# MatthewRalston/kmerdb

Measured on AMD Instinct MI355X. Metric: k-mers counted/sec at k=12, synthetic 150 bp FASTQ, higher is better.
Workload: dtype u64

## Files before the change

### kmerdb_amd/csrc/kdb_engine.hip

```cpp
#include <hip/hip_runtime.h>

#include <cmath>
#include <cstdarg>
#include <cstddef>
#include <cstdio>
#include <cstdlib>
#include <algorithm>
#include <atomic>
#include <cstring>
#include <string>
#include <thread>
#include <vector>

#include "../../include/kdbhip.h"
#include "kdb_kernels.hip.h"
#include "kdb_hist.hip.h"
#include "kdb_scatter.hip.h"
#include "kdb_scatter_host.hip.h"
#include "kdb_smallk.hip.h"
#include "kdb_probe.hip.h"
#include "kdb_gram.hip.h"
#include "kdb_pairstats.hip.h"
#include "kdb_sizefactors.hip.h"
#include "kdb_spectrum.hip.h"
// ... 67 lines not shown
struct kdb_engine {
    int k = 0, canonical = 1, n_mode = KDB_N_DROP, device = 0;
    uint64_t nbins = 0;
    unsigned long long *d_table = nullptr;
    bool owns_table = false;
    bool table_escaped = false;
    kdb::DevCounters *d_ctr = nullptr;
    unsigned long long *d_worklist = nullptr;
    size_t worklist_cap = 1u << 20;
    uint32_t *d_first_rec = nullptr; size_t first_rec_cap = 0;
    unsigned long long *d_suspects = nullptr;
    unsigned long long *sh_suspects = nullptr;
    size_t suspects_cap = 1u << 16;
    hipStream_t s_compute = nullptr, s_copy = nullptr;

    size_t stage_bytes = 64ull << 20, stage_reads = 2ull << 20;
    uint8_t *h_bases[NBUF] = {nullptr, nullptr};
    uint64_t *h_offs[NBUF] = {nullptr, nullptr};
    uint8_t *d_bases[NBUF] = {nullptr, nullptr};
    uint64_t *d_offs[NBUF] = {nullptr, nullptr};
    hipEvent_t ev_copied[NBUF] = {nullptr, nullptr}, ev_done[NBUF] = {nullptr, nullptr};
    bool inflight[NBUF] = {false, false};
    hipEvent_t busy[NBUF] = {nullptr, nullptr};
    int next_buf = 0;
    bool staging_ready = false;
    int copy_threads = 8;

    int64_t accum_bytes = -1;
    size_t acc_cap = 0, acc_reads_cap = 0;
    uint8_t *d_acc_bases[2] = {nullptr, nullptr};
    uint64_t *d_acc_offs[2] = {nullptr, nullptr};
    hipEvent_t ev_acc_done[2] = {nullptr, nullptr};
    hipEvent_t ev_acc_copied = nullptr;
    hipEvent_t ev_pin[2] = {nullptr, nullptr};
    bool pin_used[2] = {false, false};
    int pin_idx = 0;
    bool acc_inflight[2] = {false, false};
    int acc_slot = 0;
    size_t acc_nb = 0, acc_nr = 0;
    bool acc_ready = false;

    int64_t algo = 0;
    int min_len = 0;
    int smallk_old = 0;
    kdb::PagedOptions opt;
    kdb::ScatterState sc;
    int overlap = 0;
    int overlap_hist_cus = 0;
    int overlap_mask_mode = 0;
    bool compute_masked = false;
    hipStream_t s_hist = nullptr;
    kdb::OverlapState ov;
    kdb::TwoLevelPaged tp;
    int64_t oom_fallbacks = 0;
    int strand_merge = 1;
    int strand_merge_max_k = 12;
    unsigned long long *d_fwd = nullptr;
    bool strands_pending = false;

    bool tableless = false;
    uint8_t *sh_seq = nullptr; size_t sh_seq_cap = 0;
    uint64_t *sh_offs = nullptr; size_t sh_offs_cap = 0;
    unsigned long long *sh_ids = nullptr; size_t sh_ids_cap = 0;
    kdb::DevCounters *sh_ctr = nullptr;

    unsigned long long *d_acc_table = nullptr;
    uint64_t folded_files = 0, folded_total = 0;
    uint64_t d2h_bytes = 0;
    uint64_t bytes_in = 0;

    bool prof = false;
    std::vector<ProfSpan> spans;
    std::vector<hipEvent_t> ev_pool;
    double prof_ms[KDB_N_KERNELS] = {0};
    uint64_t prof_n[KDB_N_KERNELS] = {0};
};

namespace {

struct DeviceGuard {
    int prev = -1;
    explicit DeviceGuard(int dev) { if (hipGetDevice(&prev) != hipSuccess) prev = -1; (void)hipSetDevice(dev); }
    ~DeviceGuard() { if (prev >= 0) (void)hipSetDevice(prev); }
};

hipEvent_t prof_event(kdb_engine *e)
{
    hipEvent_t ev = nullptr;
    if (!e->ev_pool.empty()) { ev = e->ev_pool.back(); e->ev_pool.pop_back(); return ev; }
    if (hipEventCreate(&ev) != hipSuccess) return nullptr;
    return ev;
}

struct ProfScope {
    kdb_engine *e; int kernel; hipStream_t stream; hipEvent_t a = nullptr, b = nullptr;
    ProfScope(kdb_engine *e_, int kernel_, hipStream_t stream_ = nullptr) : e(e_), kernel(kernel_), stream(stream_ ? stream_ : e_->s_compute)
    {
        if (!e->prof) return;
        a = prof_event(e); b = prof_event(e);
        if (a) (void)hipEventRecord(a, stream);
    }
    ~ProfScope()
    {
        if (!e->prof || !a || !b) return;
        (void)hipEventRecord(b, stream);
        e->spans.push_back({a, b, kernel});
// ... 167 lines not shown
        ProfScope ps(e, KDB_KERNEL_MARK);
        const unsigned ug = (unsigned)std::min<uint64_t>((nreads + 255) / 256, 4096);
        hipLaunchKernelGGL(kdb::unmark_reads_kernel, dim3(ug), dim3(256), 0, e->s_compute, d_bases, d_offs, (uint64_t)nreads, first_is_continuation,
                           (const kdb::DevCounters *)e->d_ctr);
        marked = false;
    };
    bool no_first_rec = false;
    {
        const size_t need = ((nbytes >> kdb::FIRST_REC_SHIFT) + 2) * sizeof(uint32_t);
        if (e->first_rec_cap < need && e->d_first_rec) HIP_TRY(hipStreamSynchronize(e->s_compute));
        int grc = grow((void **)&e->d_first_rec, &e->first_rec_cap, need);
        if (grc == KDB_ERR_NOMEM) no_first_rec = true;
        else if (grc != KDB_OK) return grc;
    }
    {
        ProfScope ps(e, KDB_KERNEL_MARK);
        const dim3 grid((unsigned)((nreads + 255) / 256)), block(256);
        HIP_TRY(hipMemsetAsync(&e->d_ctr->neg_min_len, 0, kdb::PER_BATCH_WORDS * sizeof(unsigned long long), e->s_compute));
        const dim3 lgrid(grid.x < 1024u ? grid.x : 1024u);
        hipLaunchKernelGGL(kdb::lens_kernel, lgrid, block, 0, e->s_compute, d_offs, (uint64_t)nreads, (uint64_t)nbytes,
                           e->min_len > 0 ? e->min_len : e->k, first_is_continuation, e->d_ctr, e->d_first_rec);
    }
    if (nbytes == 0) return KDB_OK;
    if (nreads > 0xFFFFFFF0ull) return fail(KDB_ERR_ARG, "batch of %zu records: at most 2^32 - 16 per submit", nreads);
    e->bytes_in += nbytes;
    const kdb::RecStarts rs{d_offs, e->d_first_rec, (uint32_t)nreads, first_is_continuation ? 1u : 0u};
    int algo = (int)e->algo;
    if (algo == 0 || algo == 3) algo = 2;
    if (no_first_rec && algo == 2) { algo = 1; e->oom_fallbacks++; e->tp.table_is_zero = false; }
    const bool paged2 = algo == 2 && e->k > e->opt.one_level_max_k;
    if (!paged2 || e->n_mode == KDB_N_EXPAND || !e->opt.defer) e->tp.table_is_zero = false;
    const bool staged = e->canonical && e->strand_merge && algo == 2 && e->k <= std::min((int)e->opt.one_level_max_k, e->strand_merge_max_k) &&
                        !e->overlap && !e->smallk_old && ensure_fwd(e);
    const int canonical = staged ? 0 : e->canonical;
    unsigned long long *const table = staged ? e->d_fwd : e->d_table;
    if (staged) e->strands_pending = true;
    if (algo == 2) {
        EngineProf hook(e);
        const bool ex = e->n_mode == KDB_N_EXPAND;
        const kdb::ScBatch batch{d_bases, nbytes, rs, e->k, canonical, ex, table, e->d_ctr};
        int rc;
        if (e->k <= kdb::SMALLK_LDS_MAX_K && !e->smallk_old)
            rc = kdb::smallk_lds_count(e->s_compute, d_bases, nbytes, rs, e->k, canonical, ex, e->opt.grid, table, e->d_ctr, hook);
        else if (e->k <= kdb::SMALLK_MAX) {
            mark();
            rc = kdb::smallk_count(e->s_compute, d_bases, nbytes, e->k, canonical, ex, table, e->d_ctr, hook);
            unmark();
        }
        else if (e->k <= e->opt.one_level_max_k) {
            rc = 3;
            if (e->overlap && e->s_hist && !ex) rc = kdb::scatter_count_overlapped(e->ov, e->opt, e->s_compute, e->s_hist, batch, hook);
            if (rc == 3) {
                { const int jrc = overlap_join(e); if (jrc != KDB_OK) return jrc; }
                rc = kdb::scatter_count(e->sc, e->opt, e->s_compute, batch, hook);
            }
        }
        else {
            const size_t lost = nreads * (size_t)(e->k - 1);
            rc = kdb::twolevel_paged_count(e->tp, e->opt, e->s_compute, batch, nbytes > lost ? nbytes - lost : 0, hook);
        }
        if (rc == 2) { e->oom_fallbacks++; algo = 1; e->tp.table_is_zero = false; }
        else if (rc != 0) return fail(KDB_ERR_HIP, "LDS-histogram path failed: %s", kdb::partition_error());
    }
    if (algo == 1) {
        { const int jrc = overlap_join(e); if (jrc != KDB_OK) return jrc; }
        mark();
        {
            ProfScope ps(e, KDB_KERNEL_COUNT);
            const bool ex = (e->n_mode == KDB_N_EXPAND);
            const dim3 grid((unsigned)ntiles), block(kdb::TPB);
#define KDB_LAUNCH_DIRECT(ID, EX)                                                                              \
    hipLaunchKernelGGL((kdb::count_direct_kernel<ID, EX>), grid, block, 0, e->s_compute, d_bases, (uint64_t)nbytes, \
                       e->k, canonical, table, e->d_ctr)
            if (e->k <= 16) { if (ex) KDB_LAUNCH_DIRECT(uint32_t, true); else KDB_LAUNCH_DIRECT(uint32_t, false); }
            else            { if (ex) KDB_LAUNCH_DIRECT(uint64_t, true); else KDB_LAUNCH_DIRECT(uint64_t, false); }
#undef KDB_LAUNCH_DIRECT
        }
        unmark();
    }
    if (e->n_mode == KDB_N_EXPAND && e->d_worklist) {
        ProfScope ps(e, KDB_KERNEL_COUNT);
        hipLaunchKernelGGL(kdb::expand_worklist_kernel, dim3(1024), dim3(256), 0, e->s_compute, table, e->d_ctr, e->k, canonical);
    }
    if (e->n_mode == KDB_N_DROP) {
        ProfScope ps(e, KDB_KERNEL_MARK);
        hipLaunchKernelGGL(kdb::resolve_suspects_kernel, dim3(4), dim3(256), 0, e->s_compute, (const uint8_t *)d_bases, (uint64_t)nbytes, d_offs, (uint64_t)nreads,
                           e->k, e->d_ctr);
    }
    HIP_TRY(hipGetLastError());
    return KDB_OK;
}

int flush_pending_paged(kdb_engine *e)
{
    if (e->tp.pending == 0) return KDB_OK;
    EngineProf hook(e);
    if (kdb::twolevel_paged_flush(e->tp, e->opt, e->s_compute, e->d_table, e->d_ctr, hook)) return fail(KDB_ERR_HIP, "LDS-histogram path failed: %s", kdb::partition_error());
    return KDB_OK;
}

int check_errors(kdb_engine *e)
{
    kdb::DevCounters c;
    HIP_TRY(hipMemcpy(&c, e->d_ctr, sizeof c, hipMemcpyDeviceToHost));
    if (c.n_short)
        return fail(KDB_ERR_SHORT_READ, "%llu record(s) shorter than k=%d (reference: kmer.py:461-463 raises)",
                    c.n_short, e->k);
    if (c.bad_layout)
        return fail(KDB_ERR_ARG, "read_offsets must rise from 0 to nbytes (records tile the residue buffer exactly)");
    if (c.internal_err) {
        for (int q = 0; q < 2; q++) {
            unsigned long long hd[2] = {0, 0};
            if (e->ov.side[q] && hipMemcpy(hd, e->ov.side[q], sizeof hd, hipMemcpyDeviceToHost) == hipSuccess && hd[0] > hd[1])
                return fail(KDB_ERR_STATE, "internal: the overlapped path's side list of degenerate ids overflowed (%llu pairs for %llu places); counts are incomplete",
                            hd[0], hd[1]);
        }
        return fail(KDB_ERR_STATE, "internal: a scatter kernel ran out of its page sequence (%llu times); counts are incomplete", c.internal_err);
    }
    if (c.not_uniform)
        return fail(KDB_ERR_ARG, "kdb_submit_device_const needs records of one length (the buffer is never marked); use kdb_submit_device");
    if (c.n_bad)
        return fail(KDB_ERR_BAD_RESIDUE, "%llu residue(s) outside ACGTN%s (reference: kmer.py:309 / :170 raises)", c.n_bad,
                    e->n_mode == KDB_N_DROP ? " that no N in their window shields" : "");
    if (c.marks_seen != c.marks_set)
        return fail(KDB_ERR_BAD_RESIDUE, "the residue buffer holds %lld byte(s) with bit 7 set that are not record starts of their batch "
                                         "(not residues -- kmer.py:170 raises -- or marks left in a device buffer by a job that was aborted)",
                    (long long)(c.marks_seen - c.marks_set));
    return KDB_OK;
}

int grow(void **p, size_t *cap, size_t need_bytes)
{
    if (*cap >= need_bytes) return KDB_OK;
    if (*p) { (void)hipFree(*p); *p = nullptr; *cap = 0; }
    size_t want = need_bytes + need_bytes / 4 + 256;
    hipError_t err = hipMalloc(p, want);
    if (err != hipSuccess) { (void)hipGetLastError(); return fail(KDB_ERR_NOMEM, "hipMalloc(%zu) failed: %s", want, hipGetErrorString(err)); }
    *cap = want;
    return KDB_OK;
}

int shred_scratch(kdb_engine *e, size_t nbytes, size_t nreads)
{
    int rc;
    if ((rc = grow((void **)&e->sh_seq, &e->sh_seq_cap, nbytes + 64)) != KDB_OK) return rc;
    if ((rc = grow((void **)&e->sh_ids, &e->sh_ids_cap, nbytes * 8ull)) != KDB_OK) return rc;
    if (nreads && (rc = grow((void **)&e->sh_offs, &e->sh_offs_cap, (nreads + 1) * sizeof(uint64_t))) != KDB_OK) return rc;
// ... 51 lines not shown
    KDB_PROBE("scatter_64", R_STREAM, W_LINES_SC1, 1, 2),
    KDB_PROBE("scatter_128", R_STREAM, W_CHUNK128_SC1, 1, 2),
    KDB_PROBE("level1_64", R_STREAM, W_LINES_SC1, 1, 3),
    KDB_PROBE("level1_128", R_STREAM, W_CHUNK128_SC1, 1, 3),
    KDB_PROBE("level2_64", R_PAGES15, W_LINES_SC1, 2, 2),
    KDB_PROBE("level2_128", R_PAGES15, W_CHUNK128_SC1, 2, 2),
};
#undef KDB_PROBE
constexpr int N_PROBES = (int)(sizeof(PROBES) / sizeof(PROBES[0]));
}

namespace {
enum OptBefore { OPT_NOTHING, OPT_FLUSH_PENDING , OPT_SYNC_AND_STREAMS ,
                 OPT_SYNC , OPT_NO_STAGING  };
struct OptRow {
    const char *name;
    int64_t (*get)(kdb_engine *);
    void (*set)(kdb_engine *, int64_t) = nullptr;
    bool boolean = false;
    int64_t lo = INT64_MIN, hi = INT64_MAX;
    OptBefore before = OPT_NOTHING;
    const char *hint = "";
    int64_t multiple_of = 1;
};
#define KDB_OPT_RO(field) [](kdb_engine *e) { return (int64_t)e->field; }
#define KDB_OPT(field) KDB_OPT_RO(field), [](kdb_engine *e, int64_t v) { e->field = (decltype(e->field))v; }
const OptRow OPTIONS[] = {
    {"algo", KDB_OPT(algo), false, 0, 3, OPT_NOTHING, " (0 auto, 1 direct atomics, 2 LDS-histogram paths)"},
    {"min_len", KDB_OPT(min_len), false, 0, 64},
    {"copy_threads", KDB_OPT(copy_threads), false, 1, 64},
    {"smallk_old", KDB_OPT(smallk_old), true},
    {"accum_bytes", KDB_OPT(accum_bytes), false, -1, INT64_MAX, OPT_NO_STAGING, " (-1 auto, 0 off, else bytes)"},
    {"stage_bytes", KDB_OPT(stage_bytes), false, 4096, INT64_MAX, OPT_NO_STAGING, " (>=4096, multiple of 16)", 16},
    {"stage_reads", KDB_OPT(stage_reads), false, 1, INT64_MAX, OPT_NO_STAGING},
    {"overlap", KDB_OPT(overlap), true, 0, 1024, OPT_SYNC_AND_STREAMS},
    {"overlap_hist_cus", KDB_OPT(overlap_hist_cus), false, 0, 1024, OPT_SYNC_AND_STREAMS},
    {"overlap_mask_mode", KDB_OPT(overlap_mask_mode), false, 0, 1024, OPT_SYNC_AND_STREAMS},
    {"strand_merge", KDB_OPT(strand_merge), true, 0, 1024, OPT_SYNC},
    {"strand_merge_max_k", KDB_OPT(strand_merge_max_k), false, 1, 17, OPT_SYNC, " (1..17; never more than one_level_max_k)"},
    {"sc_grid", KDB_OPT(opt.grid), false, 0, 1024, OPT_NOTHING, " (0..1024)"},
    {"sc_lo_bits", KDB_OPT(opt.lo_bits), false, 0, kdb::SC_LO_BITS_MAX, OPT_FLUSH_PENDING, " (0 = the default of the path, 1..15)"},
    {"sc_contig_pages", KDB_OPT(opt.contig_pages), true},
    {"sc_wide_lines", KDB_OPT(opt.wide_lines), true},
    {"l1_wide_lines", KDB_OPT(opt.l1_wide), true},
    {"l2_wide_lines", KDB_OPT(opt.l2_wide), true},
    {"l1_one_round", KDB_OPT(opt.l1_one_round), true},
    {"l1_compiled_k", KDB_OPT(opt.l1k), true},
    {"one_level_max_k", KDB_OPT(opt.one_level_max_k), false, 12, kdb::SC1_K, OPT_FLUSH_PENDING, " (12 or 13)"},
    {"defer_flush", KDB_OPT(opt.defer), true},
    {"pending_budget", KDB_OPT(opt.budget_bytes), false, 0, INT64_MAX},
    {"reserve_bytes", KDB_OPT(opt.reserve_bytes), false, 0, INT64_MAX},
    {"arena_grow", KDB_OPT(opt.grow), false, 0, 2, OPT_NOTHING, " (0 never, 1 when it pays, 2 whenever the arena has filled up)"},
    {"arena_batches", KDB_OPT(opt.first_batches), false, 1, kdb::PAGED_PENDING_MAX, OPT_NOTHING, " (1..64: the arena's first size, in batches like the first one)"},
    {"k", KDB_OPT_RO(k)},
    {"arena_budget_bytes", [](kdb_engine *e) { return (int64_t)(e->opt.budget_bytes ? e->opt.budget_bytes : e->tp.budget_decided); }},
    {"free_at_sizing", KDB_OPT_RO(tp.free_at_sizing)},
    {"overlap_scatter_grid", KDB_OPT_RO(ov.grid)},
    {"oom_fallbacks", KDB_OPT_RO(oom_fallbacks)},
    {"pending_batches", KDB_OPT_RO(tp.pending)},
    {"d2h_bytes", KDB_OPT_RO(d2h_bytes)},
    {"folded_files", KDB_OPT_RO(folded_files)},
    {"bytes_in", KDB_OPT_RO(bytes_in)},
    {"arena_pages", KDB_OPT_RO(tp.arena.cap)},
    {"arena_reallocs", KDB_OPT_RO(tp.reallocs)},
    {"hist_flushes", KDB_OPT_RO(tp.flushes)},
    {"flushed_batches", KDB_OPT_RO(tp.flushed_batches)},
    {"full_flushes", KDB_OPT_RO(tp.full_flushes)},
};
#undef KDB_OPT
#undef KDB_OPT_RO
static_assert(kdb::SC_LO_BITS_MAX == 15 && kdb::SC1_K == 13 && kdb::PAGED_PENDING_MAX == 64, "the hints of sc_lo_bits, one_level_max_k and arena_batches spell these out");

const OptRow *find_option(const char *name)
{
    for (const OptRow &row : OPTIONS) if (!strcmp(name, row.name)) return &row;
    return nullptr;
}
}

namespace {

struct GramGroup { uint32_t row0, nrows; int na, nb; bool diag; };

uint32_t gram_grid_max(uint32_t nrows) { return nrows < KDB_GRAM_GRID_MANY_ROWS ? (uint32_t)KDB_GRAM_GRID_MAX : (uint32_t)KDB_GRAM_GRID_MAX_MANY_ROWS; }

void gram_launch(const GramGroup &gr, uint32_t gx, const unsigned long long *const *vecs, const kdbgram::Row *rows, uint32_t nchunks, uint32_t pstride, ulonglong2 *partials,
                 hipStream_t st)
{
    const dim3 grid(gx, gr.nrows), block(kdbgram::TPB);
    const kdbgram::Row *r = rows + gr.row0;
    ulonglong2 *p = partials + (uint64_t)gr.row0 * pstride * kdbgram::NSLOT;
#define KDB_GRAM_CASE(NA, NB, DIAG) hipLaunchKernelGGL((kdbgram::gram_kernel<NA, NB, DIAG>), grid, block, 0, st, vecs, r, nchunks, pstride, p)
    if (gr.diag) {
        switch (gr.na) {
            case 1: KDB_GRAM_CASE(1, 1, true); break;
            case 2: KDB_GRAM_CASE(2, 2, true); break;
            case 3: KDB_GRAM_CASE(3, 3, true); break;
            default: KDB_GRAM_CASE(4, 4, true); break;
        }
    } else {
        switch (gr.nb) {
            case 1: KDB_GRAM_CASE(4, 1, false); break;
            case 2: KDB_GRAM_CASE(4, 2, false); break;
            case 3: KDB_GRAM_CASE(4, 3, false); break;
            default: KDB_GRAM_CASE(4, 4, false); break;
        }
    }
#undef KDB_GRAM_CASE
}

}


extern "C" {

int kdb_abi_version(void) { return KDB_ABI_VERSION; }

const char *kdb_last_error(void) { return g_err.c_str(); }

int kdb_device_count(int *n_out)
// ... 15 lines not shown
    *out = nullptr;
    if (k < 1 || k > 17) return fail(KDB_ERR_ARG, "k=%d outside 1..17 (4^k uint64 table must fit in HBM)", k);
    if (n_mode != KDB_N_DROP && n_mode != KDB_N_EXPAND) return fail(KDB_ERR_ARG, "n_mode=%d", n_mode);
    int ndev = 0;
    HIP_TRY(hipGetDeviceCount(&ndev));
    if (device_id < 0 || device_id >= ndev) return fail(KDB_ERR_ARG, "device_id=%d but %d device(s) visible", device_id, ndev);
    DeviceGuard g(device_id);
    kdb_engine *e = new kdb_engine();
    e->k = k; e->canonical = canonicalize ? 1 : 0; e->n_mode = n_mode; e->device = device_id;
    e->nbins = 1ull << (2 * k);
    if (d_table) {
        e->d_table = (unsigned long long *)d_table;
        e->owns_table = false;
    } else {
        size_t free_b = 0, total_b = 0;
        (void)hipMemGetInfo(&free_b, &total_b);
        const unsigned long long need = e->nbins * 8ull;
        if (free_b && need > free_b) {
            delete e;
            return fail(KDB_ERR_NOMEM, "4^%d uint64 table needs %llu bytes, device has %zu free", k, need, free_b);
        }
        hipError_t me = hipMalloc((void **)&e->d_table, need);
        if (me != hipSuccess) { delete e; return fail(KDB_ERR_NOMEM, "hipMalloc(%llu) failed: %s", need, hipGetErrorString(me)); }
        e->owns_table = true;
    }
    return create_common(e, out);
}

int kdb_create_ids(int k, int canonicalize, int device_id, kdb_engine **out)
{
    if (!out) return fail(KDB_ERR_ARG, "out is NULL");
    *out = nullptr;
    if (k < 1 || k > 17) return fail(KDB_ERR_ARG, "k=%d outside 1..17", k);
    int ndev = 0;
    HIP_TRY(hipGetDeviceCount(&ndev));
    if (device_id < 0 || device_id >= ndev) return fail(KDB_ERR_ARG, "device_id=%d but %d device(s) visible", device_id, ndev);
    DeviceGuard g(device_id);
    kdb_engine *e = new kdb_engine();
    e->k = k; e->canonical = canonicalize ? 1 : 0; e->n_mode = KDB_N_DROP; e->device = device_id;
    e->nbins = 0; e->tableless = true;
    return create_common(e, out);
}

int kdb_destroy(kdb_engine *e)
{
    if (!e) return KDB_OK;
    DeviceGuard g(e->device);
    if (e->s_compute) (void)hipStreamSynchronize(e->s_compute);
    if (e->s_copy) (void)hipStreamSynchronize(e->s_copy);
    if (e->s_hist) { (void)hipStreamSynchronize(e->s_hist); (void)hipStreamDestroy(e->s_hist); }
    kdb::overlap_free(e->ov);
    kdb::scatter_free(e->sc);
    kdb::twolevel_paged_free(e->tp);
    for (auto &s : e->spans) { (void)hipEventDestroy(s.a); (void)hipEventDestroy(s.b); }
    for (auto ev : e->ev_pool) (void)hipEventDestroy(ev);
    for (int b = 0; b < NBUF; b++) {
        if (e->h_bases[b]) (void)hipHostFree(e->h_bases[b]);
        if (e->h_offs[b]) (void)hipHostFree(e->h_offs[b]);
        if (e->d_bases[b]) (void)hipFree(e->d_bases[b]);
        if (e->d_offs[b]) (void)hipFree(e->d_offs[b]);
        if (e->ev_copied[b]) (void)hipEventDestroy(e->ev_copied[b]);
        if (e->ev_done[b]) (void)hipEventDestroy(e->ev_done[b]);
    }
    for (int s2 = 0; s2 < 2; s2++) {
        if (e->d_acc_bases[s2]) (void)hipFree(e->d_acc_bases[s2]);
        if (e->d_acc_offs[s2]) (void)hipFree(e->d_acc_offs[s2]);
        if (e->ev_acc_done[s2]) (void)hipEventDestroy(e->ev_acc_done[s2]);
    }
    if (e->ev_acc_copied) (void)hipEventDestroy(e->ev_acc_copied);
    for (int s2 = 0; s2 < 2; s2++) if (e->ev_pin[s2]) (void)hipEventDestroy(e->ev_pin[s2]);
    if (e->d_worklist) (void)hipFree(e->d_worklist);
    if (e->d_suspects) (void)hipFree(e->d_suspects);
    if (e->d_first_rec) (void)hipFree(e->d_first_rec);
    if (e->sh_suspects) (void)hipFree(e->sh_suspects);
    if (e->sh_seq) (void)hipFree(e->sh_seq);
    if (e->sh_offs) (void)hipFree(e->sh_offs);
    if (e->sh_ids) (void)hipFree(e->sh_ids);
    if (e->sh_ctr) (void)hipFree(e->sh_ctr);
    if (e->d_acc_table) (void)hipFree(e->d_acc_table);
    if (e->d_fwd) (void)hipFree(e->d_fwd);
    if (e->d_ctr) (void)hipFree(e->d_ctr);
    if (e->owns_table && e->d_table) (void)hipFree(e->d_table);
    if (e->s_compute) (void)hipStreamDestroy(e->s_compute);
    if (e->s_copy) (void)hipStreamDestroy(e->s_copy);
    delete e;
    return KDB_OK;
}

int kdb_reset(kdb_engine *e)
{
    if (!e) return fail(KDB_ERR_ARG, "engine is NULL");
    DeviceGuard g(e->device);
    e->acc_nb = e->acc_nr = 0;
    kdb::twolevel_paged_drop(e->tp);
    HIP_TRY(hipStreamSynchronize(e->s_copy));
    HIP_TRY(hipStreamSynchronize(e->s_compute));
    if (e->s_hist) { HIP_TRY(hipStreamSynchronize(e->s_hist)); e->ov.last = -1; }
    if (e->nbins) HIP_TRY(hipMemsetAsync(e->d_table, 0, e->nbins * 8ull, e->s_compute));
    if (e->d_acc_table) HIP_TRY(hipMemsetAsync(e->d_acc_table, 0, e->nbins * 8ull, e->s_compute));
    if (e->strands_pending) { HIP_TRY(hipMemsetAsync(e->d_fwd, 0, e->nbins * 8ull, e->s_compute)); e->strands_pending = false; }
    e->folded_files = e->folded_total = 0;
    e->tp.table_is_zero = e->owns_table && !e->table_escaped;
    HIP_TRY(hipMemsetAsync(e->d_ctr, 0, sizeof(kdb::DevCounters), e->s_compute));
    unsigned long long wl[2] = {0, 0}, sus[2] = {0, 0};
    if (e->n_mode == KDB_N_EXPAND) {
        if (!e->d_worklist) HIP_TRY(hipMalloc((void **)&e->d_worklist, e->worklist_cap * sizeof(unsigned long long)));
        wl[0] = (unsigned long long)(uintptr_t)e->d_worklist; wl[1] = (unsigned long long)e->worklist_cap;
        HIP_TRY(hipMemcpyAsync(&e->d_ctr->wl, wl, sizeof wl, hipMemcpyHostToDevice, e->s_compute));
    } else if (!e->tableless) {
        if (!e->d_suspects) HIP_TRY(hipMalloc((void **)&e->d_suspects, e->suspects_cap * sizeof(unsigned long long)));
        sus[0] = (unsigned long long)(uintptr_t)e->d_suspects; sus[1] = (unsigned long long)e->suspects_cap;
        HIP_TRY(hipMemcpyAsync(&e->d_ctr->sus, sus, sizeof sus, hipMemcpyHostToDevice, e->s_compute));
    }
    HIP_TRY(hipStreamSynchronize(e->s_compute));
    return KDB_OK;
}

int kdb_submit_device(kdb_engine *e, void *d_bases, size_t nbytes, const void *d_read_offsets, size_t nreads)
{
    if (!e) return fail(KDB_ERR_ARG, "engine is NULL");
    if (nreads && (!d_bases || !d_read_offsets)) return fail(KDB_ERR_ARG, "NULL device buffer");
    if (((uintptr_t)d_bases & 15u) != 0) return fail(KDB_ERR_ARG, "d_bases must be 16-byte aligned");
    DeviceGuard g(e->device);
    return launch_batch(e, (uint8_t *)d_bases, nbytes, (const uint64_t *)d_read_offsets, nreads, 0, 0);
}

int kdb_submit_device_const(kdb_engine *e, const void *d_bases, size_t nbytes, const void *d_read_offsets, size_t nreads)
{
    if (!e) return fail(KDB_ERR_ARG, "engine is NULL");
    if (nreads && (!d_bases || !d_read_offsets)) return fail(KDB_ERR_ARG, "NULL device buffer");
    if (((uintptr_t)d_bases & 15u) != 0) return fail(KDB_ERR_ARG, "d_bases must be 16-byte aligned");
    DeviceGuard g(e->device);
    return launch_batch(e, (uint8_t *)const_cast<void *>(d_bases), nbytes, (const uint64_t *)d_read_offsets, nreads, 0, BATCH_CONST_INPUT);
}

static int submit_impl(kdb_engine *e, const uint8_t *bases, size_t nbytes, const uint64_t *offs, size_t nreads, bool src_pinned, bool first_continues = false)
{
    if (!e) return fail(KDB_ERR_ARG, "engine is NULL");
    if (nreads == 0) return KDB_OK;
    if (!offs || (!bases && nbytes)) return fail(KDB_ERR_ARG, "NULL host buffer");
    if (offs[nreads] < offs[0] || offs[nreads] > nbytes) return fail(KDB_ERR_ARG, "read_offsets exceed nbytes");
    DeviceGuard g(e->device);
    int rc = ensure_staging(e);
    if (rc != KDB_OK) return rc;
    if (src_pinned) {
        const int pi = e->pin_idx;
        if (!e->ev_pin[pi]) HIP_TRY(hipEventCreateWithFlags(&e->ev_pin[pi], hipEventDisableTiming));
// ... 1431 lines not shown
    const uint64_t region = 4ull << 30;
    uint8_t *src = nullptr, *dst = nullptr; uint32_t *sink = nullptr;
    hipStream_t st = nullptr;
    hipEvent_t a = nullptr, b = nullptr;
    int rc = KDB_OK;
    if (hipMalloc((void **)&src, region) != hipSuccess || hipMalloc((void **)&dst, region) != hipSuccess || hipMalloc((void **)&sink, 64) != hipSuccess) {
        (void)hipGetLastError();
        rc = fail(KDB_ERR_NOMEM, "kdb_hbm_pattern_probe: no room for two regions of 4 GiB");
    } else if (hipStreamCreateWithFlags(&st, hipStreamNonBlocking) != hipSuccess || hipEventCreate(&a) != hipSuccess || hipEventCreate(&b) != hipSuccess ||
               hipMemsetAsync(src, 1, region, st) != hipSuccess || hipMemsetAsync(dst, 0, region, st) != hipSuccess) {
        rc = fail(KDB_ERR_HIP, "kdb_hbm_pattern_probe: setup failed");
    } else {
        for (int i = 0; i < N_PROBES && rc == KDB_OK; i++) {
            const uint64_t per_step = 512ull * 8ull * ((uint64_t)PROBES[i].read_bytes + PROBES[i].write_bytes);
            const uint32_t steps = (uint32_t)(6.0e9 / (double)per_step) + 1;
            float best = 1e30f;
            for (int rep = 0; rep < 3; rep++) {
                (void)hipEventRecord(a, st);
                PROBES[i].launch(src, region, dst, region, steps, sink, st);
                (void)hipEventRecord(b, st);
                if (hipEventSynchronize(b) != hipSuccess) { rc = fail(KDB_ERR_HIP, "kdb_hbm_pattern_probe: pattern '%s' failed", PROBES[i].name); break; }
                float ms = 0;
                (void)hipEventElapsedTime(&ms, a, b);
                if (rep && ms < best) best = ms;
            }
            gb_per_s_out[i] = (double)steps * (double)per_step / 1e6 / (double)best;
        }
    }
    if (a) (void)hipEventDestroy(a);
    if (b) (void)hipEventDestroy(b);
    if (st) (void)hipStreamDestroy(st);
    if (src) (void)hipFree(src);
    if (dst) (void)hipFree(dst);
    if (sink) (void)hipFree(sink);
    return rc;
}

int kdb_set_option(kdb_engine *e, const char *name, int64_t value)
{
    if (!e || !name) return fail(KDB_ERR_ARG, "NULL argument");
    if (!strcmp(name, "sc_top_bits")) return kdb_set_option(e, "sc_lo_bits", value ? kdb::SC_LO_BITS_MAX : 0);
#ifdef KDB_SC_PROF
    if (!strcmp(name, "sc_ablate")) { int v = (int)value; (void)hipMemcpyToSymbol(HIP_SYMBOL(kdb::g_sc_ablate), &v, sizeof v); return KDB_OK; }
#endif
    const OptRow *row = find_option(name);
    if (!row || !row->set) return fail(KDB_ERR_ARG, "unknown option '%s'", name);
    if (row->before == OPT_NO_STAGING && e->staging_ready) return fail(KDB_ERR_STATE, "staging already allocated");
    if (value < row->lo || value > row->hi || value % row->multiple_of) return fail(KDB_ERR_ARG, "%s=%lld%s", name, (long long)value, row->hint);
    if (row->before == OPT_FLUSH_PENDING || (!strcmp(name, "defer_flush") && !value)) {
        DeviceGuard g(e->device);
        int rc = flush_pending_paged(e);
        if (rc != KDB_OK) return rc;
    }
    if (!strcmp(name, "pending_budget")) e->tp.budget_decided = 0;
    if (row->before != OPT_SYNC_AND_STREAMS && row->before != OPT_SYNC) { row->set(e, row->boolean ? (value ? 1 : 0) : value); return KDB_OK; }
    DeviceGuard g(e->device);
    { int rc = kdb_sync(e); if (rc != KDB_OK) return rc; }
    row->set(e, row->boolean ? (value ? 1 : 0) : value);
    return row->before == OPT_SYNC ? KDB_OK : overlap_streams(e);
}

int kdb_get_option(kdb_engine *e, const char *name, int64_t *value)
{
    if (!e || !name || !value) return fail(KDB_ERR_ARG, "NULL argument");
    if (const OptRow *row = find_option(name)) { *value = row->get(e); return KDB_OK; }
    if (!strcmp(name, "free_hbm")) {
        DeviceGuard g(e->device);
        size_t free_b = 0, total_b = 0;
        HIP_TRY(hipMemGetInfo(&free_b, &total_b));
        *value = (int64_t)free_b; return KDB_OK;
    }
    if (!strcmp(name, "arena_used_bound") || !strcmp(name, "arena_worst_case") || !strcmp(name, "arena_cursor")) {
        DeviceGuard g(e->device);
        if (!strcmp(name, "arena_cursor")) {
            uint32_t c = 0;
            HIP_TRY(hipStreamSynchronize(e->s_compute));
            if (e->tp.d_cursor && e->tp.pending) HIP_TRY(hipMemcpy(&c, e->tp.d_cursor, sizeof c, hipMemcpyDeviceToHost));
            *value = (int64_t)c; return KDB_OK;
        }
        kdb::twolevel_paged_poll(e->tp);
        *value = (int64_t)(!strcmp(name, "arena_worst_case") ? e->tp.used2 : e->tp.used2 - e->tp.slack); return KDB_OK;
    }
    {
        static const struct { const char *name; size_t off; } dev[] = {
            {"pages_bases", offsetof(kdb::DevCounters, pages_bases)}, {"lines_bases", offsetof(kdb::DevCounters, lines_bases)},
            {"pages_ids", offsetof(kdb::DevCounters, pages_ids)},     {"lines_ids", offsetof(kdb::DevCounters, lines_ids)},
            {"table_bytes", offsetof(kdb::DevCounters, table_bytes)}, {"total_kmers", offsetof(kdb::DevCounters, total_kmers)}};
        for (const auto &d : dev)
            if (!strcmp(name, d.name)) {
                DeviceGuard g(e->device);
                HIP_TRY(hipStreamSynchronize(e->s_compute));
                unsigned long long v = 0;
                HIP_TRY(hipMemcpy(&v, (const char *)e->d_ctr + d.off, sizeof v, hipMemcpyDeviceToHost));
                *value = (int64_t)v;
                return KDB_OK;
            }
    }
    return fail(KDB_ERR_ARG, "unknown option '%s'", name);
}

}
```

### kmerdb_amd/csrc/kdb_scatter_host.hip.h

```cpp
#pragma once
#include "kdb_scatter.hip.h"

namespace kdb {

constexpr int SC1_THREADS = 1024, SC1_RINGS = 1024, SC1_GRID = 256, SC1_K = 13;

struct PagedOptions {
    int grid = 0;
    int lo_bits = 0;
    int contig_pages = 1;
    int wide_lines = 1;
    int l1_wide = 1;
    int l2_wide = 1;
    int l1_one_round = 1;
    int l1k = 1;
    int one_level_max_k = SC1_K;
    int defer = 1;
    size_t budget_bytes = 0;
    size_t reserve_bytes = 0;
    int grow = 1;
    int first_batches = 8;
};

struct ScatterState {
    uint8_t *pages = nullptr; size_t cap = 0, page_bytes = 0;
    uint32_t *tag = nullptr;
    PageEntry *list = nullptr;
    uint32_t *d_bkt = nullptr; size_t bkt_cap = 0;
};

inline void page_set_free(ScatterState &st)
{
    if (st.pages) (void)hipFree(st.pages);
    if (st.tag) (void)hipFree(st.tag);
    if (st.list) (void)hipFree(st.list);
    st.pages = nullptr; st.tag = nullptr; st.list = nullptr; st.cap = 0;
}

inline int page_set_alloc(ScatterState &st, size_t npages, size_t page_bytes)
{
    if (hipMalloc((void **)&st.pages, npages * page_bytes) == hipSuccess && hipMalloc((void **)&st.tag, npages * sizeof(uint32_t)) == hipSuccess &&
        hipMalloc((void **)&st.list, npages * sizeof(PageEntry)) == hipSuccess) { st.cap = npages; st.page_bytes = page_bytes; return 0; }
    (void)hipGetLastError();
    page_set_free(st);
    return 2;
}

inline void scatter_free(ScatterState &st)
{
    page_set_free(st);
    if (st.d_bkt) (void)hipFree(st.d_bkt);
    st = ScatterState();
}

struct BktArrays { uint32_t *pages, *elems, *page_base, *slice_base; };
inline BktArrays bkt_arrays(const ScatterState &st, size_t nb) { return {st.d_bkt, st.d_bkt + nb, st.d_bkt + 2 * nb, st.d_bkt + 3 * nb + 1}; }

inline int reserve_error(int rc) { if (rc) partition_error_ref() = rc == 2 ? "scratch allocation failed" : "stream error"; return rc; }

inline int bkt_reserve(ScatterState &st, hipStream_t stream, size_t nb)
{
    if (st.bkt_cap >= nb) return 0;
    if (st.d_bkt) { if (hipStreamSynchronize(stream) != hipSuccess) return reserve_error(1); (void)hipFree(st.d_bkt); st.d_bkt = nullptr; st.bkt_cap = 0; }
    if (hipMalloc((void **)&st.d_bkt, (4 * nb + 2) * sizeof(uint32_t)) != hipSuccess) { (void)hipGetLastError(); return reserve_error(2); }
    st.bkt_cap = nb;
    return 0;
}

inline int scatter_reserve(ScatterState &st, hipStream_t stream, size_t npages, size_t nb, size_t page_bytes = SC_PAGE_BYTES)
{
    if (st.cap < npages || st.page_bytes != page_bytes) {
        if (st.pages) { if (hipStreamSynchronize(stream) != hipSuccess) return reserve_error(1); page_set_free(st); }
        if (page_set_alloc(st, npages, page_bytes)) return reserve_error(2);
    }
    return bkt_reserve(st, stream, nb);
// ... 28 lines not shown
}

struct TileGeom {
    int rings;
    uint32_t tile_pos, Gmax, page_elems;
    uint64_t ntiles_all, max_tiles;
};

inline void tile_geometry(TileGeom &g, size_t nbytes, uint32_t tile_stride, uint32_t Gmax)
{
    g.tile_pos = tile_stride * 16u;
    g.ntiles_all = ((nbytes + 15) / 16 + tile_stride - 1) / tile_stride;
    g.Gmax = Gmax;
    g.max_tiles = scatter_max_tiles(Gmax, g.tile_pos);
}

struct ScLaunch { uint32_t nt, G, extra_elems, wg_pages, npages; };

inline ScLaunch sub_batch(const TileGeom &g, uint64_t t0, int n_expand)
{
    ScLaunch L;
    L.nt = (uint32_t)((g.ntiles_all - t0) < g.max_tiles ? (g.ntiles_all - t0) : g.max_tiles);
    L.G = L.nt < g.Gmax ? L.nt : g.Gmax;
    const uint64_t wg_pos = (uint64_t)((L.nt + L.G - 1) / L.G) * g.tile_pos;
    const uint64_t floor_ = 16u * 1024u + 1024u * 64u + 2048u;
    const uint64_t extra = !n_expand ? 0 : (wg_pos / 2 > floor_ ? wg_pos / 2 : floor_);
    L.extra_elems = (uint32_t)(extra < 0x7FFFFFFFull ? extra : 0x7FFFFFFFull);
    L.wg_pages = (uint32_t)((wg_pos + L.extra_elems + g.page_elems - 1) / g.page_elems) + (uint32_t)g.rings + 1u;
    L.npages = L.G * L.wg_pages;
    return L;
}

using BasesKernel = void (*)(const uint8_t *, uint64_t, uint32_t, uint32_t, int, int, int, int, ScOut, unsigned long long *, DevCounters *, RecStarts);
using IdsKernel = void (*)(const uint8_t *, const PageEntry *, const uint32_t *, uint32_t, int, int, ScOut, DevCounters *);
struct BasesPair { BasesKernel fn[2] ; int threads; };

template <typename ID, typename EL, int RG, int CC, int RD, int TH, bool E, bool CN, int KK = 0>
inline BasesPair bases_pair() { return {{scatter_bases_kernel<ID, EL, RG, CC, RD, E, CN, KK, TH, false>, scatter_bases_kernel<ID, EL, RG, CC, RD, E, CN, KK, TH, true>}, TH}; }

template <typename ID, typename EL, int RG, int CC, int RD, int TH, int KK = 0>
inline BasesPair bases_modes(int n_expand, int canonical)
{
    if (n_expand) return canonical ? bases_pair<ID, EL, RG, CC, RD, TH, true, true, KK>() : bases_pair<ID, EL, RG, CC, RD, TH, true, false, KK>();
    return canonical ? bases_pair<ID, EL, RG, CC, RD, TH, false, true, KK>() : bases_pair<ID, EL, RG, CC, RD, TH, false, false, KK>();
}

struct ScBatch {
    const uint8_t *d_bases; size_t nbytes; RecStarts rs;
    int k, canonical, n_expand;
    unsigned long long *d_table; DevCounters *d_ctr;
};

inline int launch_bases(const BasesPair &kp, hipStream_t stream, ProfHook &prof, const ScatterState &st, int nb, const ScLaunch &L, int contig_pages,
                        const ScBatch &B, uint64_t t0, int ring_shift, int ring_bits, int sub_log2)
{
    ScOut out;
    out.pages = st.pages; out.tag = st.tag; out.extra_elems = L.extra_elems; out.wg_pages = L.wg_pages;
    out.wg_range = nullptr; out.contig = (uint32_t)contig_pages; out.wg_base = 0; out.grid = 0;
    if (hipMemsetAsync(st.tag, 0xFF, (size_t)L.npages * sizeof(uint32_t), stream) != hipSuccess ||
        hipMemsetAsync(st.d_bkt, 0, 2 * (size_t)nb * sizeof(uint32_t), stream) != hipSuccess) { partition_error_ref() = "memset failed"; return 1; }
    prof.begin_on(KDB_KERNEL_SCATTER, stream);
    for (BasesKernel fn : kp.fn)
        hipLaunchKernelGGL(fn, dim3(L.G), dim3(kp.threads), 0, stream, B.d_bases, (uint64_t)B.nbytes, (uint32_t)t0, L.nt, B.k, ring_shift, ring_bits, sub_log2, out,
                           B.d_table, B.d_ctr, B.rs);
    prof.end();
    return 0;
}

struct ScGeom : TileGeom {
    bool big; bool wide ;
    int binb, nb, sub_log2, nb_bits, lo_bits, hi_shift;
};

inline ScGeom scatter_geometry(const PagedOptions &opt, size_t nbytes, int k, uint32_t grid_default = 0)
{
    ScGeom g;
    g.big = k == SC1_K;
    g.binb = g.big ? 16 : BIN_BITS;
    g.nb = 1 << (2 * k - g.binb);
    g.rings = g.big ? SC1_RINGS : 512;
    g.page_elems = 512;
    g.lo_bits = opt.lo_bits ? opt.lo_bits : SC_LO_BITS_ONE_LEVEL;
    g.wide = !g.big && opt.wide_lines != 0;
    g.sub_log2 = 0; g.nb_bits = 2 * k - g.binb;
    while ((g.nb << g.sub_log2) < g.rings) g.sub_log2++;
    g.hi_shift = g.lo_bits + g.nb_bits;
    tile_geometry(g, nbytes, (g.big || g.wide) ? (uint32_t)SC1_THREADS - 1u : (uint32_t)SC_TILE_STRIDE,
                  opt.grid > 0 ? (uint32_t)opt.grid : (grid_default ? grid_default : (uint32_t)((g.big || g.wide) ? SC1_GRID : SC_GRID)));
    return g;
}

inline BasesPair select_one_level(const ScGeom &g, int k, int n_expand, int canonical)
{
    if (g.big) {
        if (g.lo_bits == SC_LO_BITS_ONE_LEVEL) return bases_modes<uint32_t, uint16_t, SC1_RINGS, 64, 16, SC1_THREADS, SC1_K>(n_expand, canonical);
        return bases_modes<uint32_t, uint16_t, SC1_RINGS, 64, 16, SC1_THREADS>(n_expand, canonical);
    }
    if (g.wide) {
        const bool compiled = g.lo_bits == SC_LO_BITS_ONE_LEVEL && (g.nb << g.sub_log2) == 512;
        if (compiled && k == 12) return bases_modes<uint32_t, u16w, 512, 128, 16, SC1_THREADS, 12>(n_expand, canonical);
        if (compiled && k == 11) return bases_modes<uint32_t, u16w, 512, 128, 16, SC1_THREADS, 11>(n_expand, canonical);
        if (compiled && k == 10) return bases_modes<uint32_t, u16w, 512, 128, 16, SC1_THREADS, 10>(n_expand, canonical);
        if (compiled && k == 9) return bases_modes<uint32_t, u16w, 512, 128, 16, SC1_THREADS, 9>(n_expand, canonical);
        return bases_modes<uint32_t, u16w, 512, 128, 16, SC1_THREADS>(n_expand, canonical);
    }
    if (k == 12 && g.lo_bits == SC_LO_BITS_ONE_LEVEL && g.sub_log2 == 0)
        return bases_modes<uint32_t, uint16_t, 512, 64, 16, SC_THREADS, 12>(n_expand, canonical);
    return bases_modes<uint32_t, uint16_t, 512, 64, 16, SC_THREADS>(n_expand, canonical);
}

inline int scatter_stage1(ScatterState &st, const PagedOptions &opt, hipStream_t stream, const ScGeom &g, uint64_t t0, const ScBatch &B, ProfHook &prof, ScLaunch *L)
{
    *L = sub_batch(g, t0, B.n_expand);
    if (launch_bases(select_one_level(g, B.k, B.n_expand, B.canonical), stream, prof, st, g.nb, *L, opt.contig_pages, B, t0, g.lo_bits, g.nb_bits, g.sub_log2))
        return 1;
    if (hipGetLastError() != hipSuccess) { partition_error_ref() = "paged scatter failed to launch"; return 1; }
    return 0;
}

inline int scatter_stage2(ScatterState &st, hipStream_t stream, const ScGeom &g, const ScLaunch &L, const ScBatch &B, ProfHook &prof)
{
    const uint32_t target = 512u;
    const uint32_t est_pages = (uint32_t)(((uint64_t)L.nt * g.tile_pos * 2) / SC_PAGE_BYTES) + 1u;
    uint32_t slice_pages = (est_pages + target - 1) / target;
    if (slice_pages < 128u) slice_pages = 128u;
    prof.begin_on(KDB_KERNEL_PAGE_SORT, stream);
    page_sort(stream, st, L.npages, (uint32_t)g.nb, &B.d_ctr->pages_bases, 32u, slice_pages, 256u, B.d_ctr);
    prof.end();
    prof.begin_on(KDB_KERNEL_PAGE_HIST, stream);
    hist_pass(stream, g.big, st, L.npages, (uint32_t)g.nb, slice_pages, B.d_table, g.lo_bits, g.hi_shift, 0, B.d_ctr);
    prof.end();
    if (hipGetLastError() != hipSuccess) { partition_error_ref() = "paged scatter failed to launch"; return 1; }
    return 0;
}

inline int scatter_count(ScatterState &st, const PagedOptions &opt, hipStream_t stream, const ScBatch &B, ProfHook &prof)
{
    const ScGeom g = scatter_geometry(opt, B.nbytes, B.k);
    { const int rc = scatter_reserve(st, stream, sub_batch(g, 0, B.n_expand).npages, (size_t)g.nb); if (rc) return rc; }
    for (uint64_t t0 = 0; t0 < g.ntiles_all; t0 += g.max_tiles) {
        ScLaunch L;
        if (scatter_stage1(st, opt, stream, g, t0, B, prof, &L)) return 1;
        if (scatter_stage2(st, stream, g, L, B, prof)) return 1;
    }
    return 0;
}

struct OverlapState {
    ScatterState sc[2];
    unsigned long long *side[2] = {nullptr, nullptr};
    size_t side_cap = 0;
    hipEvent_t scattered[2] = {nullptr, nullptr}, hist_done[2] = {nullptr, nullptr};
    bool used[2] = {false, false};
    int next = 0, last = -1;
    uint32_t grid = 0;
};

inline void overlap_free(OverlapState &ov)
{
    for (int j = 0; j < 2; j++) {
        scatter_free(ov.sc[j]);
        if (ov.side[j]) (void)hipFree(ov.side[j]);
        if (ov.scattered[j]) (void)hipEventDestroy(ov.scattered[j]);
        if (ov.hist_done[j]) (void)hipEventDestroy(ov.hist_done[j]);
    }
    ov = OverlapState();
}

inline int scatter_count_overlapped(OverlapState &ov, const PagedOptions &opt, hipStream_t s_scatter, hipStream_t s_hist, const ScBatch &B, ProfHook &prof)
{
    const int j = ov.next;
    ScatterState &st = ov.sc[j];
    const ScGeom g = scatter_geometry(opt, B.nbytes, B.k, ov.grid);
    if (g.ntiles_all > g.max_tiles) return 3;
    for (int q = 0; q < 2; q++) {
        if ((!ov.scattered[q] && hipEventCreateWithFlags(&ov.scattered[q], hipEventDisableTiming) != hipSuccess) ||
            (!ov.hist_done[q] && hipEventCreateWithFlags(&ov.hist_done[q], hipEventDisableTiming) != hipSuccess)) { partition_error_ref() = "event creation failed"; return 1; }
    }
    if (ov.used[j] && hipStreamWaitEvent(s_scatter, ov.hist_done[j], 0) != hipSuccess) { partition_error_ref() = "stream wait failed"; return 1; }
    const size_t npages = sub_batch(g, 0, 0).npages;
    const size_t side_need = (size_t)g.ntiles_all * (g.tile_pos / 16u + 1u) / 4u + (size_t)g.Gmax * SC_HOT;
    if ((st.cap < npages || st.bkt_cap < (size_t)g.nb) && ov.used[j] && hipEventSynchronize(ov.hist_done[j]) != hipSuccess) return reserve_error(1);
    { const int rc = scatter_reserve(st, s_scatter, npages, (size_t)g.nb); if (rc) return rc; }
    if (ov.side_cap < side_need) {
        const size_t side_new = side_need + side_need / 4;
        for (int q = 0; q < 2; q++) {
            if (ov.side[q]) { if (ov.used[q] && hipEventSynchronize(ov.hist_done[q]) != hipSuccess) return reserve_error(1); (void)hipFree(ov.side[q]); ov.side[q] = nullptr; }
            if (hipMalloc((void **)&ov.side[q], (2 + 2 * side_new) * sizeof(unsigned long long)) != hipSuccess) { (void)hipGetLastError(); ov.side_cap = 0; return reserve_error(2); }
        }
        ov.side_cap = side_new;
    }
    hipLaunchKernelGGL(hot_side_kernel, dim3(1), dim3(1), 0, s_scatter, B.d_ctr, ov.side[j], (unsigned long long)ov.side_cap);
    ScLaunch L;
    if (scatter_stage1(st, opt, s_scatter, g, 0, B, prof, &L)) return 1;
    hipLaunchKernelGGL(hot_side_kernel, dim3(1), dim3(1), 0, s_scatter, B.d_ctr, (unsigned long long *)nullptr, 0ull);
    if (hipEventRecord(ov.scattered[j], s_scatter) != hipSuccess || hipStreamWaitEvent(s_hist, ov.scattered[j], 0) != hipSuccess) { partition_error_ref() = "stream error"; return 1; }
    if (scatter_stage2(st, s_hist, g, L, B, prof)) return 1;
// ... 282 lines not shown
```

Measured before the change: 749.9 billion.

## Defer one-level page sort and histogram across several batches

```diff
diff --git a/kmerdb_amd/csrc/kdb_engine.hip b/kmerdb_amd/csrc/kdb_engine.hip
--- a/kmerdb_amd/csrc/kdb_engine.hip
+++ b/kmerdb_amd/csrc/kdb_engine.hip
@@ -143,6 +143,7 @@
     hipStream_t s_hist = nullptr;
     kdb::OverlapState ov;
     kdb::TwoLevelPaged tp;
+    kdb::OneLevelPending ol;
     int64_t oom_fallbacks = 0;
     int strand_merge = 1;
     int strand_merge_max_k = 12;
@@ -416,7 +417,8 @@
             if (e->overlap && e->s_hist && !ex) rc = kdb::scatter_count_overlapped(e->ov, e->opt, e->s_compute, e->s_hist, batch, hook);
             if (rc == 3) {
                 { const int jrc = overlap_join(e); if (jrc != KDB_OK) return jrc; }
-                rc = kdb::scatter_count(e->sc, e->opt, e->s_compute, batch, hook);
+                if (kdb::one_level_depth(e->opt, e->k) >= 2 && !(e->overlap && e->s_hist)) rc = kdb::scatter_count_deferred(e->ol, e->opt, e->s_compute, batch, hook);
+                if (rc == 3) rc = kdb::scatter_count(e->sc, e->opt, e->s_compute, batch, hook);
             }
         }
         else {
@@ -457,6 +459,10 @@
 
 int flush_pending_paged(kdb_engine *e)
 {
+    if (e->ol.used) {
+        EngineProf hook(e);
+        if (kdb::one_level_flush(e->ol, e->s_compute, e->d_ctr, hook)) return fail(KDB_ERR_HIP, "LDS-histogram path failed: %s", kdb::partition_error());
+    }
     if (e->tp.pending == 0) return KDB_OK;
     EngineProf hook(e);
     if (kdb::twolevel_paged_flush(e->tp, e->opt, e->s_compute, e->d_table, e->d_ctr, hook)) return fail(KDB_ERR_HIP, "LDS-histogram path failed: %s", kdb::partition_error());
@@ -614,20 +620,24 @@
     {"reserve_bytes", KDB_OPT(opt.reserve_bytes), false, 0, INT64_MAX},
     {"arena_grow", KDB_OPT(opt.grow), false, 0, 2, OPT_NOTHING, " (0 never, 1 when it pays, 2 whenever the arena has filled up)"},
     {"arena_batches", KDB_OPT(opt.first_batches), false, 1, kdb::PAGED_PENDING_MAX, OPT_NOTHING, " (1..64: the arena's first size, in batches like the first one)"},
+    {"one_level_defer", KDB_OPT(opt.one_level_defer), false, -1, kdb::PAGED_PENDING_MAX, OPT_FLUSH_PENDING,
+     " (-1 = 4 for k <= 12 and 0 for k = 13, 0 = sort and histogram pass per batch, 2..64 = per that many batches)"},
     {"k", KDB_OPT_RO(k)},
     {"arena_budget_bytes", [](kdb_engine *e) { return (int64_t)(e->opt.budget_bytes ? e->opt.budget_bytes : e->tp.budget_decided); }},
     {"free_at_sizing", KDB_OPT_RO(tp.free_at_sizing)},
     {"overlap_scatter_grid", KDB_OPT_RO(ov.grid)},
     {"oom_fallbacks", KDB_OPT_RO(oom_fallbacks)},
     {"pending_batches", KDB_OPT_RO(tp.pending)},
+    {"one_level_pending", KDB_OPT_RO(ol.pending)},
     {"d2h_bytes", KDB_OPT_RO(d2h_bytes)},
     {"folded_files", KDB_OPT_RO(folded_files)},
     {"bytes_in", KDB_OPT_RO(bytes_in)},
-    {"arena_pages", KDB_OPT_RO(tp.arena.cap)},
-    {"arena_reallocs", KDB_OPT_RO(tp.reallocs)},
-    {"hist_flushes", KDB_OPT_RO(tp.flushes)},
-    {"flushed_batches", KDB_OPT_RO(tp.flushed_batches)},
-    {"full_flushes", KDB_OPT_RO(tp.full_flushes)},
+    {"arena_pages", [](kdb_engine *e) { return (int64_t)(e->tp.arena.cap + e->ol.arena.cap); }},
+    {"arena_reallocs", [](kdb_engine *e) { return (int64_t)(e->tp.reallocs + e->ol.reallocs); }},
+    {"hist_flushes", [](kdb_engine *e) { return (int64_t)(e->tp.flushes + e->ol.flushes); }},
+    {"flushed_batches", [](kdb_engine *e) { return (int64_t)(e->tp.flushed_batches + e->ol.flushed_batches); }},
+    {"full_flushes", [](kdb_engine *e) { return (int64_t)(e->tp.full_flushes + e->ol.full_flushes); }},
+    {"arena_region_base", KDB_OPT_RO(ol.used)},
 };
 #undef KDB_OPT
 #undef KDB_OPT_RO
@@ -749,6 +759,7 @@
     kdb::overlap_free(e->ov);
     kdb::scatter_free(e->sc);
     kdb::twolevel_paged_free(e->tp);
+    kdb::one_level_free(e->ol);
     for (auto &s : e->spans) { (void)hipEventDestroy(s.a); (void)hipEventDestroy(s.b); }
     for (auto ev : e->ev_pool) (void)hipEventDestroy(ev);
     for (int b = 0; b < NBUF; b++) {
@@ -790,6 +801,7 @@
     DeviceGuard g(e->device);
     e->acc_nb = e->acc_nr = 0;
     kdb::twolevel_paged_drop(e->tp);
+    kdb::one_level_drop(e->ol);
     HIP_TRY(hipStreamSynchronize(e->s_copy));
     HIP_TRY(hipStreamSynchronize(e->s_compute));
     if (e->s_hist) { HIP_TRY(hipStreamSynchronize(e->s_hist)); e->ov.last = -1; }
@@ -2327,7 +2339,7 @@
         int rc = flush_pending_paged(e);
         if (rc != KDB_OK) return rc;
     }
-    if (!strcmp(name, "pending_budget")) e->tp.budget_decided = 0;
+    if (!strcmp(name, "pending_budget")) e->tp.budget_decided = e->ol.budget_decided = 0;
     if (row->before != OPT_SYNC_AND_STREAMS && row->before != OPT_SYNC) { row->set(e, row->boolean ? (value ? 1 : 0) : value); return KDB_OK; }
     DeviceGuard g(e->device);
     { int rc = kdb_sync(e); if (rc != KDB_OK) return rc; }
diff --git a/kmerdb_amd/csrc/kdb_scatter_host.hip.h b/kmerdb_amd/csrc/kdb_scatter_host.hip.h
--- a/kmerdb_amd/csrc/kdb_scatter_host.hip.h
+++ b/kmerdb_amd/csrc/kdb_scatter_host.hip.h
@@ -20,7 +20,10 @@
     size_t reserve_bytes = 0;
     int grow = 1;
     int first_batches = 8;
-};
+    int one_level_defer = -1;
+};
+constexpr int ONE_LEVEL_DEPTH = 4;
+inline int one_level_depth(const PagedOptions &opt, int k) { return opt.one_level_defer >= 0 ? opt.one_level_defer : (k <= 12 ? ONE_LEVEL_DEPTH : 0); }
 
 struct ScatterState {
     uint8_t *pages = nullptr; size_t cap = 0, page_bytes = 0;
@@ -155,13 +158,14 @@
 };
 
 inline int launch_bases(const BasesPair &kp, hipStream_t stream, ProfHook &prof, const ScatterState &st, int nb, const ScLaunch &L, int contig_pages,
-                        const ScBatch &B, uint64_t t0, int ring_shift, int ring_bits, int sub_log2)
+                        const ScBatch &B, uint64_t t0, int ring_shift, int ring_bits, int sub_log2, int64_t region = -1)
 {
     ScOut out;
     out.pages = st.pages; out.tag = st.tag; out.extra_elems = L.extra_elems; out.wg_pages = L.wg_pages;
     out.wg_range = nullptr; out.contig = (uint32_t)contig_pages; out.wg_base = 0; out.grid = 0;
-    if (hipMemsetAsync(st.tag, 0xFF, (size_t)L.npages * sizeof(uint32_t), stream) != hipSuccess ||
-        hipMemsetAsync(st.d_bkt, 0, 2 * (size_t)nb * sizeof(uint32_t), stream) != hipSuccess) { partition_error_ref() = "memset failed"; return 1; }
+    if (region >= 0) { out.pages += (size_t)region * st.page_bytes; out.tag += (size_t)region; }
+    else if (hipMemsetAsync(st.tag, 0xFF, (size_t)L.npages * sizeof(uint32_t), stream) != hipSuccess ||
+             hipMemsetAsync(st.d_bkt, 0, 2 * (size_t)nb * sizeof(uint32_t), stream) != hipSuccess) { partition_error_ref() = "memset failed"; return 1; }
     prof.begin_on(KDB_KERNEL_SCATTER, stream);
     for (BasesKernel fn : kp.fn)
         hipLaunchKernelGGL(fn, dim3(L.G), dim3(kp.threads), 0, stream, B.d_bases, (uint64_t)B.nbytes, (uint32_t)t0, L.nt, B.k, ring_shift, ring_bits, sub_log2, out,
@@ -246,6 +250,115 @@
         if (scatter_stage1(st, opt, stream, g, t0, B, prof, &L)) return 1;
         if (scatter_stage2(st, stream, g, L, B, prof)) return 1;
     }
+    return 0;
+}
+
+struct OneLevelPending {
+    ScatterState arena;
+    size_t used = 0;
+    size_t est_pages = 0;
+    size_t tags_dirty = 0;
+    int pending = 0;
+    int k = 0, nb = 0, lo_bits = 0, hi_shift = 0; bool big = false;
+    unsigned long long *d_table = nullptr;
+    size_t budget_decided = 0;
+    bool grow_failed = false;
+    uint64_t reallocs = 0, flushes = 0, flushed_batches = 0, full_flushes = 0;
+};
+constexpr size_t ARENA_BYTES_PER_PAGE = SC_PAGE_BYTES + sizeof(uint32_t) + sizeof(PageEntry);
+
+inline void one_level_free(OneLevelPending &ol) { scatter_free(ol.arena); ol = OneLevelPending(); }
+
+inline void one_level_drop(OneLevelPending &ol)
+{
+    if (ol.used > ol.tags_dirty) ol.tags_dirty = ol.used;
+    ol.used = 0; ol.est_pages = 0; ol.pending = 0;
+}
+
+inline size_t one_level_est_pages(const ScGeom &g, const ScLaunch &L) { return (size_t)(((uint64_t)L.nt * g.tile_pos * 2) / SC_PAGE_BYTES) + 1u; }
+
+inline int one_level_flush(OneLevelPending &ol, hipStream_t stream, DevCounters *d_ctr, ProfHook &prof)
+{
+    if (ol.used == 0) { one_level_drop(ol); return 0; }
+    const size_t target = 512;
+    size_t slice_pages = (ol.est_pages + target - 1) / target;
+    if (slice_pages < 128) slice_pages = 128;
+    if (slice_pages > (1u << 17) - 1u) slice_pages = (1u << 17) - 1u;
+    if (hipMemsetAsync(ol.arena.d_bkt, 0, 2 * (size_t)ol.nb * sizeof(uint32_t), stream) != hipSuccess) { partition_error_ref() = "memset failed"; return 1; }
+    prof.begin_on(KDB_KERNEL_PAGE_SORT, stream);
+    page_sort(stream, ol.arena, (uint32_t)ol.used, (uint32_t)ol.nb, &d_ctr->pages_bases, 32u, (uint32_t)slice_pages, 256u, d_ctr);
+    prof.end();
+    prof.begin_on(KDB_KERNEL_PAGE_HIST, stream);
+    hist_pass(stream, ol.big, ol.arena, (uint32_t)ol.used, (uint32_t)ol.nb, (uint32_t)slice_pages, ol.d_table, ol.lo_bits, ol.hi_shift, 0, d_ctr);
+    prof.end();
+    ol.flushes++; ol.flushed_batches += (uint64_t)ol.pending;
+    one_level_drop(ol);
+    if (hipGetLastError() != hipSuccess) { partition_error_ref() = "histogram pass over the one-level arena failed to launch"; return 1; }
+    return 0;
+}
+
+inline int one_level_room(OneLevelPending &ol, const PagedOptions &opt, hipStream_t stream, int depth, size_t need, size_t nb, DevCounters *d_ctr, ProfHook &prof)
+{
+    if (ol.arena.cap && ol.used + need <= ol.arena.cap && ol.arena.bkt_cap >= nb) return 0;
+    const bool filled_up = ol.used != 0;
+    if (filled_up) { ol.full_flushes++; if (one_level_flush(ol, stream, d_ctr, prof)) return 1; }
+    if (opt.budget_bytes == 0 && ol.budget_decided == 0) {
+        size_t free_b = 0, total_b = 0;
+        (void)hipMemGetInfo(&free_b, &total_b);
+        ol.budget_decided = free_b / 100 * 85;
+        if (opt.reserve_bytes && ol.budget_decided + opt.reserve_bytes > free_b) ol.budget_decided = free_b > opt.reserve_bytes ? free_b - opt.reserve_bytes : 0;
+        if (ol.budget_decided > (192ull << 30)) ol.budget_decided = 192ull << 30;
+        if (ol.budget_decided == 0) ol.budget_decided = 1;
+    }
+    size_t budget_pages = (opt.budget_bytes ? opt.budget_bytes : ol.budget_decided) / ARENA_BYTES_PER_PAGE;
+    if (ol.grow_failed && budget_pages > ol.arena.cap) budget_pages = ol.arena.cap;
+    size_t want = (size_t)depth * need;
+    if (want > budget_pages) want = budget_pages;
+    const bool too_small = ol.arena.cap < 2 * need, grow = filled_up && want >= ol.arena.cap + ol.arena.cap / 4;
+    if (too_small || grow) {
+        if (want < 2 * need) { ol.budget_decided = 0; return 3; }
+        if (hipStreamSynchronize(stream) != hipSuccess) return reserve_error(1);
+        page_set_free(ol.arena);
+        ol.reallocs++;
+        if (page_set_alloc(ol.arena, want, SC_PAGE_BYTES) != 0) {
+            ol.grow_failed = true;
+            if (page_set_alloc(ol.arena, 2 * need, SC_PAGE_BYTES) != 0) { ol.tags_dirty = 0; return 3; }
+        }
+        ol.tags_dirty = ol.arena.cap;
+    }
+    const int rc = bkt_reserve(ol.arena, stream, nb);
+    return rc == 2 ? 3 : rc;
+}
+
+inline int one_level_begin_cycle(OneLevelPending &ol, hipStream_t stream)
+{
+    if (ol.tags_dirty > ol.arena.cap) ol.tags_dirty = ol.arena.cap;
+    if (ol.tags_dirty && hipMemsetAsync(ol.arena.tag, 0xFF, ol.tags_dirty * sizeof(uint32_t), stream) != hipSuccess) { partition_error_ref() = "memset failed"; return 1; }
+    ol.tags_dirty = 0;
+    return 0;
+}
+
+inline int scatter_count_deferred(OneLevelPending &ol, const PagedOptions &opt, hipStream_t stream, const ScBatch &B, ProfHook &prof)
+{
+    const ScGeom g = scatter_geometry(opt, B.nbytes, B.k);
+    const int depth = one_level_depth(opt, B.k);
+    if (ol.used && (ol.k != B.k || ol.nb != g.nb || ol.lo_bits != g.lo_bits || ol.hi_shift != g.hi_shift || ol.big != g.big || ol.d_table != B.d_table)) {
+        if (one_level_flush(ol, stream, B.d_ctr, prof)) return 1;
+    }
+    { const int rc = one_level_room(ol, opt, stream, depth, sub_batch(g, 0, B.n_expand).npages, (size_t)g.nb, B.d_ctr, prof); if (rc) return rc; }
+    ol.k = B.k; ol.nb = g.nb; ol.lo_bits = g.lo_bits; ol.hi_shift = g.hi_shift; ol.big = g.big; ol.d_table = B.d_table;
+    const BasesPair kp = select_one_level(g, B.k, B.n_expand, B.canonical);
+    for (uint64_t t0 = 0; t0 < g.ntiles_all; t0 += g.max_tiles) {
+        const ScLaunch L = sub_batch(g, t0, B.n_expand);
+        if (ol.used + L.npages > ol.arena.cap) { ol.full_flushes++; if (one_level_flush(ol, stream, B.d_ctr, prof)) return 1; }
+        if (ol.used == 0 && one_level_begin_cycle(ol, stream)) return 1;
+        if (launch_bases(kp, stream, prof, ol.arena, g.nb, L, opt.contig_pages, B, t0, g.lo_bits, g.nb_bits, g.sub_log2, (int64_t)ol.used)) return 1;
+        if (hipGetLastError() != hipSuccess) { partition_error_ref() = "paged scatter failed to launch"; return 1; }
+        ol.used += L.npages;
+        ol.est_pages += one_level_est_pages(g, L);
+    }
+    ol.pending++;
+    if (ol.pending >= depth) return one_level_flush(ol, stream, B.d_ctr, prof);
     return 0;
 }
 
```

Result: faster. 791.1 billion, median of 6 (+5.5%).
